# vlc-robot/robot-3dlotus

Measured on AMD Instinct MI355X. Metric: keystep-samples/sec (train fwd+bwd) 3D-LOTUS GemBench, higher is better.
Workload: dtype f32; 1 GPU; 3D-LOTUS v1 (68.18M params), 16 key-step clouds x 4096 pts per GPU, fwd+loss+bwd, train mode (dropout on), fp32 exact (MFMA f32); global_batch=16, parallelism=dp1, rccl_ranks=0

## Files before the change

### robot-3dlotus_amd/csrc/gemm.hip

```cpp
#include "gemm_common.h"
#include <stdlib.h>
#include <type_traits>

namespace LOTUS_NS {


template <int R, bool KC, int BK>
struct GTile {
  static constexpr int kLd = KC ? BK + 4 : R;
  static constexpr int kFloats = KC ? R * (BK + 4) : BK * R;
};

template <int BM, int BN, int BK, bool A_KC, bool B_KC, bool SUM_A>
__device__ __forceinline__ void gemm_slab(const float* __restrict__ As, const float* __restrict__ Bs, int wr0, int wc0,
                                          f32x16 (&acc)[BM / 64][BN / 64], float (&asum)[BM / 64]) {
  constexpr int TM = BM / 64, TN = BN / 64, KS = BK / 2;
  const int l31 = threadIdx.x & 31, h = (threadIdx.x >> 5) & 1;
  float a[TM][KS], b[TN][KS];
#pragma unroll
  for (int tm = 0; tm < TM; ++tm) {
    if (A_KC) {
      const float* row = As + (wr0 + tm * 32 + l31) * GTile<BM, true, BK>::kLd + h * KS;
#pragma unroll
      for (int q = 0; q < KS / 4; ++q) {
        const float4 v = ld4(row + 4 * q);
        a[tm][4 * q] = v.x; a[tm][4 * q + 1] = v.y; a[tm][4 * q + 2] = v.z; a[tm][4 * q + 3] = v.w;
      }
    } else {
#pragma unroll
      for (int s2 = 0; s2 < KS; ++s2) a[tm][s2] = As[(h * KS + s2) * BM + wr0 + tm * 32 + l31];
    }
  }
#pragma unroll
  for (int tn = 0; tn < TN; ++tn) {
    if (B_KC) {
      const float* row = Bs + (wc0 + tn * 32 + l31) * GTile<BN, true, BK>::kLd + h * KS;
#pragma unroll
      for (int q = 0; q < KS / 4; ++q) {
        const float4 v = ld4(row + 4 * q);
        b[tn][4 * q] = v.x; b[tn][4 * q + 1] = v.y; b[tn][4 * q + 2] = v.z; b[tn][4 * q + 3] = v.w;
      }
    } else {
#pragma unroll
      for (int s2 = 0; s2 < KS; ++s2) b[tn][s2] = Bs[(h * KS + s2) * BN + wc0 + tn * 32 + l31];
    }
  }
#pragma unroll
  for (int s2 = 0; s2 < KS; ++s2) {
#pragma unroll
    for (int tm = 0; tm < TM; ++tm) {
      if (SUM_A) asum[tm] += a[tm][s2];
#pragma unroll
      for (int tn = 0; tn < TN; ++tn) acc[tm][tn] = __builtin_amdgcn_mfma_f32_32x32x2f32(a[tm][s2], b[tn][s2], acc[tm][tn], 0, 0, 0);
    }
  }
}


__device__ __forceinline__ float4 zsel(bool ok, float4 v) {
  return make_float4(ok ? v.x : 0.f, ok ? v.y : 0.f, ok ? v.z : 0.f, ok ? v.w : 0.f);
}

template <int BM, int BN, int BK, bool A_KC, bool B_KC, bool SUM_A, bool FAST, int PREC = 0, typename EA = float, typename EB = float,
          typename EC = float, int RD = 1, bool TAP = false>
__global__ __launch_bounds__(256) void gemm_kernel(GemmP p) {
  const EA* __restrict__ pA = static_cast<const EA*>(p.A);
  const EB* __restrict__ pB = static_cast<const EB*>(p.B);
  const int* __restrict__ a_rows = TAP ? p.a_rows : nullptr;
  constexpr int TM = BM / 64, TN = BN / 64;
  constexpr int A4 = BM * BK / 4 / 256, B4 = BN * BK / 4 / 256;
  static_assert(A4 >= 1 && B4 >= 1, "tile too small");
  static_assert(PREC == 0 || ((!SUM_A || !A_KC) && BK % 16 == 0 && (A_KC || A4 % 2 == 0) && (B_KC || B4 % 2 == 0)),
                "bf16 path: operands contiguous along their non-reduction index are staged as k pairs; the bias-gradient "
                "sums are taken from the fp32 staging registers of such an A operand");
  constexpr int AF = PREC ? BTile<BM, BK, PREC>::kWords : GTile<BM, A_KC, BK>::kFloats;
  constexpr int BF = PREC ? BTile<BN, BK, PREC>::kWords : GTile<BN, B_KC, BK>::kFloats;
  constexpr int WN = BN / 2, SLD = WN + 4;
  constexpr int LDSF = (2 * AF + 2 * BF) > (4 * 32 * SLD) ? (2 * AF + 2 * BF) : (4 * 32 * SLD);
  __shared__ __attribute__((aligned(16))) float smem[LDSF];
  float* As = smem;
  float* Bs = smem + 2 * AF;

  const int tid = threadIdx.x, wave = tid >> 6;
  int bx = blockIdx.x, by = blockIdx.y, bz = blockIdx.z;
  if (gridDim.z > 1 && (gridDim.z & 7) == 0) {
    const int tiles = gridDim.x * gridDim.y;
    const int id = (blockIdx.z * gridDim.y + blockIdx.y) * gridDim.x + blockIdx.x;
    const int xcd = id & 7, slot = id >> 3;
    bz = xcd + 8 * (slot / tiles);
    const int t = slot - (slot / tiles) * tiles;
    by = t / (int)gridDim.x;
    bx = t - by * (int)gridDim.x;
  } else {
    const int nbx = gridDim.x, total = nbx * gridDim.y;
    const int lin = by * nbx + bx, xcd = lin & 7, slot = lin >> 3;
    const int q = total >> 3, r = total & 7;
    const int t = xcd * q + min(xcd, r) + slot;
    by = t / nbx;
    bx = t - by * nbx;
  }
  const int m0 = by * BM, n0 = bx * BN;
  if constexpr (TAP) {
    const int tap = m0 / p.tap_rows;
    if (m0 - tap * p.tap_rows >= p.tap_cnt[tap]) return;
    pB += (long)(p.b_tap_mirror ? 26 - tap : tap) * p.b_tap_stride;
  }
  auto arow = [&](int r) { r = min(r, p.M - 1); return TAP ? a_rows[r] : r; };
  const int kbeg = bz * p.klen;
  const int kend = min(p.K, kbeg + p.klen);
  const int wr0 = (wave >> 1) * (BM / 2), wc0 = (wave & 1) * (BN / 2);

  f32x16 acc[TM][TN];
#pragma unroll
  for (int i = 0; i < TM; ++i)
#pragma unroll
    for (int j = 0; j < TN; ++j)
#pragma unroll
      for (int r = 0; r < 16; ++r) acc[i][j][r] = 0.f;
  float asum[TM];
#pragma unroll
  for (int i = 0; i < TM; ++i) asum[i] = 0.f;

  float bsum[4] = {0.f, 0.f, 0.f, 0.f};
  Raw4<EA> rring_a[RD][A4];
  Raw4<EB> rring_b[RD][B4];
  auto gload = [&](Raw4<EA> (&rra)[A4], Raw4<EB> (&rrb)[B4], int k0) {
#pragma unroll
    for (int t = 0; t < A4; ++t) {
      const int f = tid + t * 256;
      if (A_KC) {
        const int row = f / (BK / 4), kq = f % (BK / 4);
        if (FAST) {
          const int k = k0 + kq * 4;
          rra[t] = rsel(k < kend, ldraw(pA + (long)arow(m0 + row) * p.lda + min(k, p.K - 4)));
        } else {
          rra[t] = toraw(load4_guard(pA, p.lda, m0 + row, k0 + kq * 4, p.M, kend, p.a_vec), pA);
        }
      } else {
        const int f2 = PREC ? tid + (t >> 1) * 256 : f;
        const int kr = PREC ? (f2 / (BM / 4)) * 2 + (t & 1) : f / (BM / 4), iq = f2 % (BM / 4);
        if (FAST) {
          const int k = k0 + kr;
          rra[t] = rsel(k < kend, ldraw(pA + (long)min(k, p.K - 1) * p.lda + min(m0 + iq * 4, p.M - 4)));
        } else {
          rra[t] = toraw(load4_guard(pA, p.lda, k0 + kr, m0 + iq * 4, kend, p.M, p.a_vec), pA);
        }
      }
    }
#pragma unroll
    for (int t = 0; t < B4; ++t) {
      const int f = tid + t * 256;
      if (B_KC) {
        const int row = f / (BK / 4), kq = f % (BK / 4);
        if (FAST) {
          const int k = k0 + kq * 4;
          rrb[t] = rsel(k < kend, ldraw(pB + (long)min(n0 + row, p.N - 1) * p.ldb + min(k, p.K - 4)));
        } else {
          rrb[t] = toraw(load4_guard(pB, p.ldb, n0 + row, k0 + kq * 4, p.N, kend, p.b_vec), pB);
        }
      } else {
        const int f2 = PREC ? tid + (t >> 1) * 256 : f;
        const int kr = PREC ? (f2 / (BN / 4)) * 2 + (t & 1) : f / (BN / 4), jq = f2 % (BN / 4);
        if (FAST) {
          const int k = k0 + kr;
          rrb[t] = rsel(k < kend, ldraw(pB + (long)min(k, p.K - 1) * p.ldb + min(n0 + jq * 4, p.N - 4)));
        } else {
          rrb[t] = toraw(load4_guard(pB, p.ldb, k0 + kr, n0 + jq * 4, kend, p.N, p.b_vec), pB);
        }
      }
    }
  };
  auto lstore = [&](const Raw4<EA> (&rra)[A4], const Raw4<EB> (&rrb)[B4], float* Ad, float* Bd) {
    float4 ra[A4], rb[B4];
#pragma unroll
    for (int t = 0; t < A4; ++t) ra[t] = unraw(rra[t]);
#pragma unroll
    for (int t = 0; t < B4; ++t) rb[t] = unraw(rrb[t]);
    if (PREC) {
      unsigned* Aw = reinterpret_cast<unsigned*>(Ad);
      unsigned* Bw = reinterpret_cast<unsigned*>(Bd);
      using TA = BTile<BM, BK, PREC ? PREC : 1>;
      using TB = BTile<BN, BK, PREC ? PREC : 1>;
      if (A_KC) {
#pragma unroll
        for (int t = 0; t < A4; ++t) {
          const int f = tid + t * 256, row = f / (BK / 4), kq = f % (BK / 4);
          unsigned h0, l0, h1, l1;
          split_bf16(ra[t].x, ra[t].y, h0, l0);
          split_bf16(ra[t].z, ra[t].w, h1, l1);
          *reinterpret_cast<uint2*>(&Aw[row * TA::kLdW + kq * 2]) = make_uint2(h0, h1);
          if (PREC == 3) *reinterpret_cast<uint2*>(&Aw[TA::kPlaneW + row * TA::kLdW + kq * 2]) = make_uint2(l0, l1);
        }
      } else {
#pragma unroll
        for (int t = 0; t + 1 < A4; t += 2) {
          const int f2 = tid + (t >> 1) * 256, kr2 = f2 / (BM / 4), iq = f2 % (BM / 4);
          const float va[4] = {ra[t].x, ra[t].y, ra[t].z, ra[t].w}, vb[4] = {ra[t + 1].x, ra[t + 1].y, ra[t + 1].z, ra[t + 1].w};
          unsigned hw[4], lw[4];
#pragma unroll
          for (int e = 0; e < 4; ++e) split_bf16(va[e], vb[e], hw[e], lw[e]);
          if (SUM_A && bx == 0) {
#pragma unroll
            for (int e = 0; e < 4; ++e) bsum[e] += va[e] + vb[e];
          }
          const int rot = (iq >> 2) & 3;
          rot4(hw, rot);
          if (PREC == 3) rot4(lw, rot);
#pragma unroll
          for (int e = 0; e < 4; ++e) {
            const int row = iq * 4 + ((e + rot) & 3);
            Aw[row * TA::kLdW + kr2] = hw[e];
            if (PREC == 3) Aw[TA::kPlaneW + row * TA::kLdW + kr2] = lw[e];
          }
        }
      }
      if (B_KC) {
#pragma unroll
        for (int t = 0; t < B4; ++t) {
          const int f = tid + t * 256, row = f / (BK / 4), kq = f % (BK / 4);
          unsigned h0, l0, h1, l1;
          split_bf16(rb[t].x, rb[t].y, h0, l0);
          split_bf16(rb[t].z, rb[t].w, h1, l1);
          *reinterpret_cast<uint2*>(&Bw[row * TB::kLdW + kq * 2]) = make_uint2(h0, h1);
          if (PREC == 3) *reinterpret_cast<uint2*>(&Bw[TB::kPlaneW + row * TB::kLdW + kq * 2]) = make_uint2(l0, l1);
        }
      } else {
#pragma unroll
        for (int t = 0; t + 1 < B4; t += 2) {
          const int f2 = tid + (t >> 1) * 256, kr2 = f2 / (BN / 4), jq = f2 % (BN / 4);
          const float va[4] = {rb[t].x, rb[t].y, rb[t].z, rb[t].w}, vb[4] = {rb[t + 1].x, rb[t + 1].y, rb[t + 1].z, rb[t + 1].w};
          unsigned hw[4], lw[4];
#pragma unroll
          for (int e = 0; e < 4; ++e) split_bf16(va[e], vb[e], hw[e], lw[e]);
          const int rot = (jq >> 2) & 3;
          rot4(hw, rot);
          if (PREC == 3) rot4(lw, rot);
#pragma unroll
          for (int e = 0; e < 4; ++e) {
            const int row = jq * 4 + ((e + rot) & 3);
            Bw[row * TB::kLdW + kr2] = hw[e];
            if (PREC == 3) Bw[TB::kPlaneW + row * TB::kLdW + kr2] = lw[e];
          }
        }
      }
      return;
    }
#pragma unroll
    for (int t = 0; t < A4; ++t) {
      const int f = tid + t * 256;
      const float v[4] = {ra[t].x, ra[t].y, ra[t].z, ra[t].w};
      if (A_KC) {
        const int row = f / (BK / 4), kq = f % (BK / 4);
        st4(&Ad[row * GTile<BM, true, BK>::kLd + kq * 4], ra[t]);
      } else {
        const int kr = f / (BM / 4), iq = f % (BM / 4);
        st4(&Ad[kr * BM + iq * 4], ra[t]);
      }
    }
#pragma unroll
    for (int t = 0; t < B4; ++t) {
      const int f = tid + t * 256;
      const float v[4] = {rb[t].x, rb[t].y, rb[t].z, rb[t].w};
      if (B_KC) {
        const int row = f / (BK / 4), kq = f % (BK / 4);
        st4(&Bd[row * GTile<BN, true, BK>::kLd + kq * 4], rb[t]);
      } else {
        const int kr = f / (BN / 4), jq = f % (BN / 4);
        st4(&Bd[kr * BN + jq * 4], rb[t]);
      }
    }
  };

  const EA* pa[A4];
  const EB* pb[B4];
  if (FAST) {
#pragma unroll
    for (int t = 0; t < A4; ++t) {
      const int f = tid + t * 256;
      if (A_KC) pa[t] = pA + (long)arow(m0 + f / (BK / 4)) * p.lda + (f % (BK / 4)) * 4;
      else if (PREC) pa[t] = pA + (long)(((tid + (t >> 1) * 256) / (BM / 4)) * 2 + (t & 1)) * p.lda + min(m0 + ((tid + (t >> 1) * 256) % (BM / 4)) * 4, p.M - 4);
      else pa[t] = pA + (long)(f / (BM / 4)) * p.lda + min(m0 + (f % (BM / 4)) * 4, p.M - 4);
    }
#pragma unroll
    for (int t = 0; t < B4; ++t) {
      const int f = tid + t * 256;
      if (B_KC) pb[t] = pB + (long)min(n0 + f / (BK / 4), p.N - 1) * p.ldb + (f % (BK / 4)) * 4;
      else if (PREC) pb[t] = pB + (long)(((tid + (t >> 1) * 256) / (BN / 4)) * 2 + (t & 1)) * p.ldb + min(n0 + ((tid + (t >> 1) * 256) % (BN / 4)) * 4, p.N - 4);
      else pb[t] = pB + (long)(f / (BN / 4)) * p.ldb + min(n0 + (f % (BN / 4)) * 4, p.N - 4);
    }
  }
  auto gload_full = [&](Raw4<EA> (&rra)[A4], Raw4<EB> (&rrb)[B4], int k0) {
#pragma unroll
    for (int t = 0; t < A4; ++t) rra[t] = ldraw(pa[t] + (A_KC ? (long)k0 : (long)k0 * p.lda));
#pragma unroll
    for (int t = 0; t < B4; ++t) rrb[t] = ldraw(pb[t] + (B_KC ? (long)k0 : (long)k0 * p.ldb));
  };

  auto slab = [&](int cur) {
    if (PREC) gemm_slab_bf16<BM, BN, BK, PREC ? PREC : 1>(reinterpret_cast<const unsigned*>(As + cur * AF), reinterpret_cast<const unsigned*>(Bs + cur * BF), wr0, wc0, acc);
    else if (SUM_A && bx == 0) gemm_slab<BM, BN, BK, A_KC, B_KC, true>(As + cur * AF, Bs + cur * BF, wr0, wc0, acc, asum);
    else gemm_slab<BM, BN, BK, A_KC, B_KC, false>(As + cur * AF, Bs + cur * BF, wr0, wc0, acc, asum);
  };
  auto simple_loop = [&]() {
    gload(rring_a[0], rring_b[0], kbeg);
    lstore(rring_a[0], rring_b[0], As, Bs);
    __syncthreads();
    int cur = 0;
    for (int k0 = kbeg; k0 < kend; k0 += BK) {
      if (FAST && k0 + 2 * BK <= kend) gload_full(rring_a[0], rring_b[0], k0 + BK);
      else gload(rring_a[0], rring_b[0], k0 + BK);
      __builtin_amdgcn_sched_barrier(0);
      slab(cur);
      __builtin_amdgcn_sched_barrier(0);
      cur ^= 1;
      lstore(rring_a[0], rring_b[0], As + cur * AF, Bs + cur * BF);
      __syncthreads();
    }
  };
  if constexpr (RD == 1 || !FAST) {
    if (kbeg < kend) simple_loop();
  } else if (kend - kbeg < RD * BK) {
    if (kbeg < kend) simple_loop();
  } else {
#pragma unroll
    for (int d = 0; d < RD; ++d) gload_full(rring_a[d], rring_b[d], kbeg + d * BK);
    lstore(rring_a[0], rring_b[0], As, Bs);
    __syncthreads();
    int cur = 0, k0 = kbeg;
    for (; k0 + 2 * RD * BK <= kend; k0 += RD * BK) {
#pragma unroll
      for (int d = 0; d < RD; ++d) {
        gload_full(rring_a[d], rring_b[d], k0 + (d + RD) * BK);
        __builtin_amdgcn_sched_barrier(0);
        slab(cur);
        __builtin_amdgcn_sched_barrier(0);
        cur ^= 1;
        lstore(rring_a[(d + 1) % RD], rring_b[(d + 1) % RD], As + cur * AF, Bs + cur * BF);
        __syncthreads();
      }
    }
#pragma unroll
    for (int d = 0; d < 2 * RD; ++d) {
      const int kk = k0 + d * BK;
      if (kk < kend) {
        if (d < RD && kk + RD * BK < kend) {
          if (kk + (RD + 1) * BK <= kend) gload_full(rring_a[d], rring_b[d], kk + RD * BK);
          else gload(rring_a[d], rring_b[d], kk + RD * BK);
        }
        __builtin_amdgcn_sched_barrier(0);
        slab(cur);
        __builtin_amdgcn_sched_barrier(0);
        cur ^= 1;
        if (kk + BK < kend) lstore(rring_a[(d + 1) % RD], rring_b[(d + 1) % RD], As + cur * AF, Bs + cur * BF);
        __syncthreads();
      }
    }
  }

  const bool fused = FAST && p.cnt != nullptr && gridDim.z > 1;
  EC* __restrict__ C = static_cast<EC*>(p.C) + (long)bz * p.part_stride;
  float* __restrict__ Cp = fused ? p.part + (long)bz * p.part_stride : nullptr;
  if (FAST) {
    float* st = smem + wave * (32 * SLD);
    const int l31 = tid & 31, hh = (tid >> 5) & 1, lane = tid & 63;
    constexpr int LPR = WN / 4;
    constexpr int RPI = 64 / LPR;
    __syncthreads();
#pragma unroll
    for (int tm = 0; tm < TM; ++tm) {
#pragma unroll
      for (int tn = 0; tn < TN; ++tn)
#pragma unroll
        for (int r = 0; r < 16; ++r) st[((r & 3) + 8 * (r >> 2) + 4 * hh) * SLD + tn * 32 + l31] = acc[tm][tn][r];
      __syncthreads();
      const int c4 = lane % LPR;
      const int col = n0 + wc0 + c4 * 4;
      if (col < p.N) {
#pragma unroll
        for (int it = 0; it < 32 / RPI; ++it) {
          const int rl = it * RPI + lane / LPR;
          const int row = m0 + wr0 + tm * 32 + rl;
          if (row < p.M) {
            const long o = (long)row * p.ldc + col;
            const float4 a4 = ld4(st + rl * SLD + c4 * 4);
            if (fused) {
              st_agent4(Cp + o, a4);
            } else {
              float v[4] = {a4.x, a4.y, a4.z, a4.w};
              gemm_epilogue4(p, C, o, col, v);
            }
          }
        }
      }
      __syncthreads();
    }
  } else {
#pragma unroll
    for (int tm = 0; tm < TM; ++tm)
#pragma unroll
      for (int tn = 0; tn < TN; ++tn) {
        const int col = n0 + acc_col(wc0, tn);
        if (col >= p.N) continue;
        const float bv = p.bias ? p.bias[col] : 0.f;
#pragma unroll
        for (int r = 0; r < 16; ++r) {
          const int row = m0 + acc_row(wr0, tm, r);
          if (row >= p.M) continue;
          const long o = (long)row * p.ldc + col;
          float v = acc[tm][tn][r] + bv;
          if (p.pre) st1(p.pre + o, v);
          v = act_f(v, p.act);
          if (p.mulpre) v *= act_grad_f(ld1(p.mulpre + o), p.dact);
          if (p.drop_thresh) v *= dropout_scale(p.drop_seed, (unsigned long long)o, p.drop_thresh, p.drop_inv_keep);
          if (p.residual) v += ld1(p.residual + o);
          st1(C + o, v);
        }
      }
  }
  if (SUM_A && PREC) {
    __syncthreads();
    if (p.bias_part && bx == 0) {
      float4* red = reinterpret_cast<float4*>(smem);
      red[tid] = make_float4(bsum[0], bsum[1], bsum[2], bsum[3]);
      __syncthreads();
      if (tid < BM) {
        constexpr int G = 256 / (BM / 4);
        float sacc = 0.f;
#pragma unroll
        for (int g = 0; g < G; ++g) {
          const float4 v = red[g * (BM / 4) + (tid >> 2)];
          sacc += (tid & 3) == 0 ? v.x : (tid & 3) == 1 ? v.y : (tid & 3) == 2 ? v.z : v.w;
        }
        if (m0 + tid < p.M) __hip_atomic_store(p.bias_part + (long)bz * p.bias_stride + m0 + tid, sacc, __ATOMIC_RELAXED, __HIP_MEMORY_SCOPE_AGENT);
      }
    }
  } else if (SUM_A) {
    if (p.bias_part && bx == 0 && (wave & 1) == 0) {
#pragma unroll
      for (int tm = 0; tm < TM; ++tm) {
        float s = asum[tm] + __shfl_xor(asum[tm], 32, 64);
        const int i = m0 + wr0 + tm * 32 + (tid & 31);
        if ((tid & 32) == 0 && i < p.M) __hip_atomic_store(p.bias_part + (long)bz * p.bias_stride + i, s, __ATOMIC_RELAXED, __HIP_MEMORY_SCOPE_AGENT);
      }
    }
  }
  if (FAST && fused) splitk_fused_tail<SUM_A, BM, BN, EC>(p, bx, by, m0, n0, tid);
}

template <typename T>
__global__ __launch_bounds__(256) void reduce_parts_kernel(const T* __restrict__ part, T* __restrict__ out, long n,
                                                           long stride, int nz, int accumulate) {
  __shared__ float4 red[16][16];
  const int q = threadIdx.x & 15, zl = threadIdx.x >> 4;
  const long e = ((long)blockIdx.x * 16 + q) * 4;
  float4 s = make_float4(0.f, 0.f, 0.f, 0.f);
  if (e + 3 < n) {
    for (int z = zl; z < nz; z += 16) {
      const float4 v = ld4(part + (long)z * stride + e);
      s.x += v.x; s.y += v.y; s.z += v.z; s.w += v.w;
    }
  } else if (e < n) {
    float t[4] = {0.f, 0.f, 0.f, 0.f};
    for (int z = zl; z < nz; z += 16)
      for (int k = 0; k < 4 && e + k < n; ++k) t[k] += ld1(part + (long)z * stride + e + k);
    s = make_float4(t[0], t[1], t[2], t[3]);
  }
  red[zl][q] = s;
  __syncthreads();
  if (zl == 0 && e < n) {
    float4 t = red[0][q];
    for (int k = 1; k < 16; ++k) {
      t.x += red[k][q].x; t.y += red[k][q].y; t.z += red[k][q].z; t.w += red[k][q].w;
    }
    const float tv[4] = {t.x, t.y, t.z, t.w};
    for (int k = 0; k < 4 && e + k < n; ++k) st1(out + e + k, accumulate ? ld1(out + e + k) + tv[k] : tv[k]);
  }
}

int lotus_reduce_parts(const float* part, float* out, long n, long stride, int nz, int accumulate, hipStream_t st) {
  if (n <= 0) return LOTUS_OK;
  LOTUS_LAUNCH(reduce_parts_kernel<float>, dim3(cdiv(n, 64)), dim3(256), 0, st, part, out, n, stride, nz, accumulate);
  LOTUS_LAUNCH_CHECK("lotus_reduce_parts");
  return LOTUS_OK;
}

extern "C" int lotus_sum_slabs(const act_t* part, act_t* out, long n, long stride, int nz, void* stream) {
  LOTUS_CHECK_ARG(part && out && n >= 0 && nz >= 1, "lotus_sum_slabs: bad arguments");
  if (n <= 0) return LOTUS_OK;
  LOTUS_LAUNCH(reduce_parts_kernel<act_t>, dim3(cdiv(n, 64)), dim3(256), 0, (hipStream_t)stream, part, out, n, stride, nz, 0);
  LOTUS_LAUNCH_CHECK("lotus_sum_slabs");
  return LOTUS_OK;
}

__global__ __launch_bounds__(256) void sum_slabs_ld_kernel(const act_t* __restrict__ part, act_t* __restrict__ out, int rows, int cols,
                                                           long out_ld, long stride, int nz) {
  const int c4 = cols / 4;
  const long i = (long)blockIdx.x * 256 + threadIdx.x;
  if (i >= (long)rows * c4) return;
  const int r = (int)(i / c4), q = (int)(i % c4);
  const act_t* src = part + (long)r * cols + 4 * q;
  float4 s = ld4(src);
  int z = 1;
  for (; z + 3 < nz; z += 4) {
    const float4 v0 = ld4(src + (long)z * stride), v1 = ld4(src + (long)(z + 1) * stride);
    const float4 v2 = ld4(src + (long)(z + 2) * stride), v3 = ld4(src + (long)(z + 3) * stride);
    s.x = (((s.x + v0.x) + v1.x) + v2.x) + v3.x; s.y = (((s.y + v0.y) + v1.y) + v2.y) + v3.y;
    s.z = (((s.z + v0.z) + v1.z) + v2.z) + v3.z; s.w = (((s.w + v0.w) + v1.w) + v2.w) + v3.w;
  }
  for (; z < nz; ++z) {
    const float4 v = ld4(src + (long)z * stride);
    s.x += v.x; s.y += v.y; s.z += v.z; s.w += v.w;
  }
  st4(out + (long)r * out_ld + 4 * q, s);
}

extern "C" int lotus_sum_slabs_ld(const act_t* part, act_t* out, int rows, int cols, long out_ld, long stride, int nz, void* stream) {
  LOTUS_CHECK_ARG(part && out && rows >= 0 && cols > 0 && cols % 4 == 0 && out_ld % 4 == 0 && stride % 4 == 0 && nz >= 1,
                  "lotus_sum_slabs_ld: bad arguments (cols, out_ld and stride must be multiples of 4)");
  if (rows == 0) return LOTUS_OK;
  LOTUS_LAUNCH(sum_slabs_ld_kernel, dim3(cdiv((long)rows * (cols / 4), 256)), dim3(256), 0, (hipStream_t)stream, part, out, rows, cols,
               out_ld, stride, nz);
  LOTUS_LAUNCH_CHECK("lotus_sum_slabs_ld");
  return LOTUS_OK;
}

static inline int vec_ok(const void* p, long ld) { return (((uintptr_t)p) % 16 == 0) && (ld % 4 == 0); }

#define GEMM_KALIGN 64

#define GEMM_GO_RD(BM_, BN_, BK_, PREC_, grid_, RD_)                                                                             \
  do {                                                                                                                           \
    using TB_ = std::conditional_t<SUM_A, act_t, float>;                                                                         \
                            \
    auto note_ = [&] { lotus_note_dense_route(1, BM_, BN_, BK_, nz, FAST, FAST && p.cnt && nz > 1, RD_); };                      \
    if constexpr (LOTUS_ACT_IS_BF16 && !SUM_A) {                                                                                 \
      if (p.b_act) {                       \
        if constexpr (PREC_ == 1 && FAST) {                                                                                      \
          note_();                                                                                                               \
          if (p.c_float) LOTUS_LAUNCH((gemm_kernel<BM_, BN_, BK_, A_KC, B_KC, SUM_A, FAST, PREC_, act_t, act_t, float, RD_>), grid_, block, 0, st, p); \
          else LOTUS_LAUNCH((gemm_kernel<BM_, BN_, BK_, A_KC, B_KC, SUM_A, FAST, PREC_, act_t, act_t, act_t, RD_>), grid_, block, 0, st, p); \
        }                                                                                                                        \
      } else if (p.c_float) {                                                                                                    \
        note_();                                                                                                                 \
        LOTUS_LAUNCH((gemm_kernel<BM_, BN_, BK_, A_KC, B_KC, SUM_A, FAST, PREC_, act_t, TB_, float, RD_>), grid_, block, 0, st, p); \
      } else {                                                                                                                   \
        note_();                                                                                                                 \
        LOTUS_LAUNCH((gemm_kernel<BM_, BN_, BK_, A_KC, B_KC, SUM_A, FAST, PREC_, act_t, TB_, act_t, RD_>), grid_, block, 0, st, p); \
      }                                                                                                                          \
    } else {                                                                                                                     \
      note_();                                                                                                                   \
      LOTUS_LAUNCH((gemm_kernel<BM_, BN_, BK_, A_KC, B_KC, SUM_A, FAST, PREC_, act_t, TB_, float, RD_>), grid_, block, 0, st, p);      \
    }                                                                                                                            \
  } while (0)
#define GEMM_GO(BM_, BN_, BK_, PREC_, grid_) GEMM_GO_RD(BM_, BN_, BK_, PREC_, grid_, 1)

constexpr long kF32RingMaxBlocks = 8192;
constexpr int kBf16RingMaxRows = 8192;

template <bool A_KC, bool B_KC, bool SUM_A, bool FAST>
static int launch_gemm_t(GemmP& p, int nz, hipStream_t st) {
  const long blocks64 = (long)cdiv(p.M, 64) * cdiv(p.N, 64);
  dim3 block(256);
  dim3 g64(cdiv(p.N, 64), cdiv(p.M, 64), nz);
  const int g_prec = p.prec;
  if (g_prec && SUM_A && FAST && !A_KC && !B_KC) {
    if constexpr (SUM_A && !A_KC && !B_KC && FAST) {
      if (g_prec == 1) {
        if constexpr (LOTUS_ACT_IS_BF16) {
          if (p.K <= kBf16RingMaxRows) GEMM_GO_RD(64, 64, 32, 1, g64, 4);
          else GEMM_GO(64, 64, 32, 1, g64);
        } else {
          GEMM_GO(64, 64, 32, 1, g64);
        }
      } else if constexpr (!LOTUS_ACT_IS_BF16) GEMM_GO(64, 64, 32, 3, g64);
    }
    LOTUS_LAUNCH_CHECK("lotus_gemm(bf16 wgrad)");
    return LOTUS_OK;
  }
  if (p.b_act && !(LOTUS_ACT_IS_BF16 && g_prec == 1 && !SUM_A && FAST && (A_KC || p.M % 4 == 0))) {
    lotus_set_error("lotus_linear: bf16 weight shadows (precision 5) need the bf16-storage build and 16-byte aligned operands whose "
                    "widths are multiples of 4");
    return LOTUS_E_UNSUPPORTED;
  }
  if (g_prec && !SUM_A && FAST && (A_KC || p.M % 4 == 0)) {
    if constexpr (!SUM_A && FAST) {
      if (g_prec == 1) {
        if constexpr (LOTUS_ACT_IS_BF16) {
          if (p.M <= kBf16RingMaxRows) GEMM_GO_RD(64, 64, 32, 1, g64, 4);
          else GEMM_GO(64, 64, 32, 1, g64);
        } else GEMM_GO(64, 64, 32, 1, g64);
      } else if constexpr (!LOTUS_ACT_IS_BF16) {
        GEMM_GO(64, 64, 32, 3, g64);
      }
    }
    LOTUS_LAUNCH_CHECK("lotus_gemm(bf16)");
    return LOTUS_OK;
  }
  if constexpr (LOTUS_ACT_IS_BF16) {
    GEMM_GO(64, 64, 32, 0, g64);
  } else {
    const long blocks_eff = p.tap_rows ? blocks64 / 2 : blocks64;
    const int bk = SUM_A ? 32 : (blocks_eff * nz <= 512 ? 64 : (blocks_eff * nz <= 2048 ? 32 : 16));
    const int rd = SUM_A ? 1 : (blocks_eff * nz <= kF32RingMaxBlocks ? 2 : 1);
    if (p.tap_rows) {
      if constexpr (A_KC && !SUM_A && FAST && !LOTUS_ACT_IS_BF16) {
        lotus_note_dense_route(1, 64, 64, bk, nz, FAST, 0, 2);
        if (bk == 64) LOTUS_LAUNCH((gemm_kernel<64, 64, 64, A_KC, B_KC, SUM_A, FAST, 0, act_t, float, float, 2, true>), g64, block, 0, st, p);
        else if (bk == 32) LOTUS_LAUNCH((gemm_kernel<64, 64, 32, A_KC, B_KC, SUM_A, FAST, 0, act_t, float, float, 2, true>), g64, block, 0, st, p);
        else LOTUS_LAUNCH((gemm_kernel<64, 64, 16, A_KC, B_KC, SUM_A, FAST, 0, act_t, float, float, 2, true>), g64, block, 0, st, p);
        LOTUS_LAUNCH_CHECK("lotus_gemm(tap-grouped)");
        return LOTUS_OK;
      } else {
        lotus_set_error("lotus_gemm: tap-grouped products need k-contiguous, 16-byte aligned fp32 rows");
        return LOTUS_E_UNSUPPORTED;
      }
    }
    if (rd == 2 && bk == 64) GEMM_GO_RD(64, 64, 64, 0, g64, 2);
    else if (rd == 2 && bk == 16) GEMM_GO_RD(64, 64, 16, 0, g64, 2);
    else if (rd == 2) GEMM_GO_RD(64, 64, 32, 0, g64, 2);
    else if (bk == 64) GEMM_GO(64, 64, 64, 0, g64);
    else if (bk == 32) GEMM_GO(64, 64, 32, 0, g64);
    else GEMM_GO(64, 64, 16, 0, g64);
  }
  LOTUS_LAUNCH_CHECK("lotus_gemm");
  return LOTUS_OK;
}

template <bool A_KC, bool B_KC>
static bool fast_ok(const GemmP& p) {
  const bool a_ok = p.a_vec && (A_KC ? (p.K % 4 == 0 && p.K >= 4) : (p.M % 4 == 0 && p.M >= 4));
  const bool b_ok = p.b_vec && (B_KC ? (p.K % 4 == 0 && p.K >= 4) : (p.N % 4 == 0 && p.N >= 4));
  const bool c_ok = p.N % 4 == 0 && p.ldc % 4 == 0 && p.part_stride % 4 == 0 && vec_ok(p.C, p.ldc) &&
                    (!p.bias || ((uintptr_t)p.bias) % 16 == 0) && (!p.residual || ((uintptr_t)p.residual) % 16 == 0) &&
                    (!p.pre || ((uintptr_t)p.pre) % 16 == 0) && (!p.mulpre || ((uintptr_t)p.mulpre) % 16 == 0) &&
                    (!p.part || ((uintptr_t)p.part) % 16 == 0);
  return a_ok && b_ok && c_ok;
}

template <bool A_KC, bool B_KC, bool SUM_A>
static int launch_gemm(GemmP& p, int nz, hipStream_t st) {
  const bool a_ok = p.a_vec && (A_KC ? (p.K % 4 == 0 && p.K >= 4) : (p.M % 4 == 0 && p.M >= 4));
  const bool b_ok = p.b_vec && (B_KC ? (p.K % 4 == 0 && p.K >= 4) : (p.N % 4 == 0 && p.N >= 4));
  const bool c_ok = p.N % 4 == 0 && p.ldc % 4 == 0 && p.part_stride % 4 == 0 && vec_ok(p.C, p.ldc) &&
                    (!p.bias || ((uintptr_t)p.bias) % 16 == 0) && (!p.residual || ((uintptr_t)p.residual) % 16 == 0) &&
                    (!p.pre || ((uintptr_t)p.pre) % 16 == 0) && (!p.mulpre || ((uintptr_t)p.mulpre) % 16 == 0);
  if (a_ok && b_ok && c_ok) {
    if constexpr (A_KC || SUM_A) {
      const int rc = launch_gemm_dma(p, A_KC ? (B_KC ? 0 : 1) : 2, nz, st);
      if (rc != LOTUS_GEMM_DMA_NA) return rc;
    }
    return launch_gemm_t<A_KC, B_KC, SUM_A, true>(p, nz, st);
  }
  return launch_gemm_t<A_KC, B_KC, SUM_A, false>(p, nz, st);
}

static void set_drop(GemmP& p, float drop_p, unsigned long long seed) {
  p.drop_seed = seed;
  lotus_drop_setup(drop_p, &p.drop_thresh, &p.drop_inv_keep);
}

__global__ void splitk_epilogue_kernel(GemmP p, const float* __restrict__ part, long stride, int nz) {
  const int n4 = p.N / 4;
  const long total4 = (long)p.M * n4;
  for (long i = (long)blockIdx.x * blockDim.x + threadIdx.x; i < total4; i += (long)gridDim.x * blockDim.x) {
    const int row = (int)(i / n4), col = (int)(i % n4) * 4;
    const long o = (long)row * p.ldc + col;
    float4 s4 = ld4(part + o);
    for (int z = 1; z < nz; ++z) {
      const float4 v = ld4(part + (long)z * stride + o);
      s4.x += v.x; s4.y += v.y; s4.z += v.z; s4.w += v.w;
    }
    float v[4] = {s4.x, s4.y, s4.z, s4.w};
    if (p.bias) {
      const float4 b = ld4(p.bias + col);
      v[0] += b.x; v[1] += b.y; v[2] += b.z; v[3] += b.w;
    }
    if (p.pre) st4(p.pre + o, make_float4(v[0], v[1], v[2], v[3]));
#pragma unroll
    for (int e = 0; e < 4; ++e) v[e] = act_f(v[e], p.act);
    if (p.mulpre) {
      const float4 m4 = ld4(p.mulpre + o);
      const float mv[4] = {m4.x, m4.y, m4.z, m4.w};
#pragma unroll
      for (int e = 0; e < 4; ++e) v[e] *= act_grad_f(mv[e], p.dact);
    }
    if (p.drop_thresh) {
      float dm[4];
      dropout_scale4(p.drop_seed, (unsigned long long)o, p.drop_thresh, p.drop_inv_keep, dm);
#pragma unroll
      for (int e = 0; e < 4; ++e) v[e] *= dm[e];
    }
    if (p.residual) {
      const float4 r4 = ld4(p.residual + o);
      v[0] += r4.x; v[1] += r4.y; v[2] += r4.z; v[3] += r4.w;
    }
    st4(static_cast<act_t*>(p.C) + o, make_float4(v[0], v[1], v[2], v[3]));
  }
}

static int fwd_splits(int M, int N, int K) {
  const long blocks = (long)cdiv(M, 64) * cdiv(N, 64);
  int nz = 1;
  while (nz < 16 && blocks * nz < 512 && K / (nz * 2) >= 384) nz *= 2;
  return nz;
}

#define LOTUS_SPLITK_MAX_TILES 4096

static bool splitk_fused_enabled() {
  static int on = -1;
  if (on < 0) { const char* e = getenv("LOTUS_SPLITK_FUSED"); on = (e && e[0] == '0') ? 0 : 1; }
  return on != 0;
}

template <bool A_KC, bool B_KC>
static int run_gemm_splitk(GemmP& p, void* workspace, size_t workspace_bytes, unsigned* counters, hipStream_t st) {
  if (!splitk_fused_enabled()) counters = nullptr;
  const int nz = (p.N % 4 == 0 && p.ldc == p.N) ? fwd_splits(p.M, p.N, p.K) : 1;
  const size_t need = (size_t)nz * p.M * p.N * sizeof(float);
  if (nz == 1 || !workspace || workspace_bytes < need || ((uintptr_t)workspace) % 16) return launch_gemm<A_KC, B_KC, false>(p, 1, st);
  const int klen = cdiv(cdiv(p.K, nz), GEMM_KALIGN) * GEMM_KALIGN;
  const long tiles = (long)cdiv(p.M, 64) * cdiv(p.N, 64);
  if (counters && tiles <= LOTUS_SPLITK_MAX_TILES) {
    GemmP q = p;
    q.part = (float*)workspace; q.part_stride = (long)p.M * p.N; q.cnt = counters; q.klen = klen;
    if (fast_ok<A_KC, B_KC>(q)) return launch_gemm<A_KC, B_KC, false>(q, nz, st);
  }
  GemmP q = p;
  q.C = workspace; q.c_float = 1; q.part_stride = (long)p.M * p.N;
  q.bias = nullptr; q.residual = nullptr; q.pre = nullptr; q.mulpre = nullptr; q.act = LOTUS_ACT_NONE; q.drop_thresh = 0;
  q.klen = klen;
  StopEventOnLast stop_ev;
  int rc = launch_gemm<A_KC, B_KC, false>(q, nz, st);
  if (rc) return rc;
  const long total4 = (long)p.M * p.N / 4;
  int g = cdiv(total4, 256);
  stop_ev.last();
  LOTUS_LAUNCH(splitk_epilogue_kernel, dim3(g > 2048 ? 2048 : g), dim3(256), 0, st, p, (const float*)workspace,
                     (long)p.M * p.N, nz);
  LOTUS_LAUNCH_CHECK("lotus_gemm(split-K epilogue)");
  return LOTUS_OK;
}

int lotus_conv_tap_gemm(int mode, const act_t* x, const float* w, float* part, const int* tg_in, const int* tg_cnt, int n64,
                        int src_rows, int cin, int cout, hipStream_t st) {
  if constexpr (LOTUS_ACT_IS_BF16) {
    return LOTUS_E_UNSUPPORTED;
  } else {
    GemmP p;
    memset(&p, 0, sizeof(p));
    p.A = x; p.B = w; p.C = part;
    p.M = 27 * n64;
    p.N = mode == 0 ? cout : cin;
    p.K = mode == 0 ? cin : cout;
    p.lda = p.K; p.ldb = 27L * cin; p.ldc = p.N;
    p.act = LOTUS_ACT_NONE;
    p.klen = cdiv(p.K, GEMM_KALIGN) * GEMM_KALIGN;
    p.a_vec = vec_ok(x, p.K); p.b_vec = vec_ok(w, cin) && cin % 4 == 0; p.prec = 0;
    p.drop_inv_keep = 1.f;
    p.a_rows = tg_in; p.tap_cnt = tg_cnt; p.tap_rows = n64; p.b_tap_mirror = mode == 1; p.b_tap_stride = cin;
    p.a_src_rows = src_rows;
    {
      GemmP q = p;
      const int rc = launch_gemm_dma_tap(q, mode, st);
      if (rc != LOTUS_GEMM_DMA_NA) return rc;
    }
    if (!(fast_ok<true, true>(p))) {
      lotus_set_error("lotus_subm_conv(tap-grouped): rows, weights and the partial slab must be 16-byte aligned with widths that are multiples of 4");
      return LOTUS_E_UNSUPPORTED;
    }
    return mode == 0 ? launch_gemm<true, true, false>(p, 1, st) : launch_gemm<true, false, false>(p, 1, st);
  }
}

extern "C" {

size_t lotus_splitk_counters_bytes(void) { return (size_t)(LOTUS_SPLITK_MAX_TILES + 64) * sizeof(unsigned); }
size_t lotus_bn_counters_offset(void) { return (size_t)LOTUS_SPLITK_MAX_TILES * sizeof(unsigned); }

size_t lotus_linear_workspace(int M, int N, int K) {
  const int a = fwd_splits(M, N, K), b = fwd_splits(M, K, N);
  const size_t wa = a > 1 ? (size_t)a * M * N * sizeof(float) : 0, wb = b > 1 ? (size_t)b * M * K * sizeof(float) : 0;
  return wa > wb ? wa : wb;
}

int lotus_linear_fwd(const act_t* x, const float* w, const float* bias, const act_t* residual, act_t* y,
                     act_t* pre, int M, int N, int K, int act, float drop_p, unsigned long long drop_seed,
                     int precision, void* workspace, size_t workspace_bytes, void* counters, void* stream) {
  LOTUS_CHECK_ARG(x && w && y && M >= 0 && N > 0 && K > 0, "lotus_linear_fwd: bad arguments");
  const int w_shadow = precision == 5;
  LOTUS_CHECK_ARG(!w_shadow || LOTUS_ACT_IS_BF16, "lotus_linear_fwd: precision 5 (bf16 weight shadow) exists in the bf16-storage build only");
  if (w_shadow) precision = 1;
  LOTUS_CHECK_ARG(precision == 0 || precision == 1 || precision == 3, "lotus_linear_fwd: precision must be 0, 1 or 3 (5 with bf16 weights)");
  LOTUS_CHECK_ARG(!(LOTUS_ACT_IS_BF16 && precision == 3), "lotus_linear_fwd: bf16x3 operands (precision 3) are not built for bf16 activation storage; use 1 (bf16) or 0");
  if (M == 0) return LOTUS_OK;
  GemmP p;
  memset(&p, 0, sizeof(p));
  p.A = x; p.B = w; p.C = y; p.M = M; p.N = N; p.K = K;
  p.lda = K; p.ldb = K; p.ldc = N;
  p.bias = bias; p.residual = residual; p.pre = pre; p.act = act;
  p.klen = cdiv(K, GEMM_KALIGN) * GEMM_KALIGN;
  p.a_vec = vec_ok(x, K); p.b_vec = vec_ok(w, K); p.prec = precision; p.b_act = w_shadow;
  set_drop(p, drop_p, drop_seed);
  return run_gemm_splitk<true, true>(p, workspace, workspace_bytes, (unsigned*)counters, (hipStream_t)stream);
}

int lotus_linear_dgrad(const act_t* dy, const float* w, act_t* dx, const act_t* pre, const act_t* add, int M,
                       int N, int K, int act, float drop_p, unsigned long long drop_seed, int precision, void* workspace,
                       size_t workspace_bytes, void* counters, void* stream) {
  LOTUS_CHECK_ARG(dy && w && dx && M >= 0 && N > 0 && K > 0, "lotus_linear_dgrad: bad arguments");
  const int w_shadow = precision == 5;
  LOTUS_CHECK_ARG(!w_shadow || LOTUS_ACT_IS_BF16, "lotus_linear_dgrad: precision 5 (bf16 weight shadow) exists in the bf16-storage build only");
  if (w_shadow) precision = 1;
  LOTUS_CHECK_ARG(precision == 0 || precision == 1 || precision == 3, "lotus_linear_dgrad: precision must be 0, 1 or 3 (5 with bf16 weights)");
  LOTUS_CHECK_ARG(!(LOTUS_ACT_IS_BF16 && precision == 3), "lotus_linear_dgrad: bf16x3 operands (precision 3) are not built for bf16 activation storage; use 1 (bf16) or 0");
  if (M == 0) return LOTUS_OK;
  GemmP p;
  memset(&p, 0, sizeof(p));
  p.A = dy; p.B = w; p.C = dx; p.M = M; p.N = K; p.K = N;
  p.lda = N; p.ldb = K; p.ldc = K;
  p.act = LOTUS_ACT_NONE;
  p.mulpre = pre; p.dact = act; p.residual = add;
  p.klen = cdiv(N, GEMM_KALIGN) * GEMM_KALIGN;
  p.a_vec = vec_ok(dy, N); p.b_vec = vec_ok(w, K); p.prec = precision; p.b_act = w_shadow;
  set_drop(p, drop_p, drop_seed);
  return run_gemm_splitk<true, false>(p, workspace, workspace_bytes, (unsigned*)counters, (hipStream_t)stream);
}

int lotus_layernorm_bwd(const act_t* dy, const act_t* x, const float* mean, const float* rstd, const float* gamma, const act_t* add,
                        act_t* dx, float* dgamma, float* dbeta, int M, int C, int accumulate, act_t* dz, float drop_p,
                        unsigned long long drop_seed, void* workspace, size_t workspace_bytes, void* stream);
int lotus_layernorm_bwd_parts(int M, int C);
int lotus_linear_dgrad_ln(const act_t* dy, const float* w, const act_t* x, const float* mean, const float* rstd, const float* gamma,
                          const act_t* add, act_t* dx, act_t* dn, act_t* dz, float dz_p, unsigned long long dz_seed, int M, int N,
                          int K, int precision, void* workspace, size_t workspace_bytes, void* counters, void* ln_workspace,
                          size_t ln_workspace_bytes, int* nparts, void* stream) {
  LOTUS_CHECK_ARG(dy && w && x && mean && rstd && gamma && dx && dn && nparts && ln_workspace && M >= 0 && N > 0 && K > 0,
                  "lotus_linear_dgrad_ln: bad arguments");
  LOTUS_CHECK_ARG(!dz || dz_p > 0.f, "lotus_linear_dgrad_ln: dz needs dz_p > 0");
  if (M == 0) { *nparts = 0; return LOTUS_OK; }
  if (precision == 0 && !LOTUS_ACT_IS_BF16 && (size_t)cdiv(M, 128) * 2 * K * sizeof(float) <= ln_workspace_bytes) {
    GemmP p;
    memset(&p, 0, sizeof(p));
    p.A = dy; p.B = w; p.C = dx; p.M = M; p.N = K; p.K = N;
    p.lda = N; p.ldb = K; p.ldc = K;
    p.act = LOTUS_ACT_NONE; p.residual = add;
    p.klen = cdiv(N, GEMM_KALIGN) * GEMM_KALIGN;
    p.a_vec = vec_ok(dy, N); p.b_vec = vec_ok(w, K); p.prec = 0;
    set_drop(p, dz ? dz_p : 0.f, dz_seed);
    p.ln_x = x; p.ln_mean = mean; p.ln_rstd = rstd; p.ln_gamma = gamma; p.ln_part = (float*)ln_workspace; p.ln_dz = dz;
    if (p.a_vec && p.b_vec && vec_ok(dx, K) && vec_ok(x, K) && (!add || vec_ok(add, K))) {
      const int rc = launch_gemm_dma(p, 1, 1, (hipStream_t)stream);
      if (rc != LOTUS_GEMM_DMA_NA) { *nparts = cdiv(M, 128); return rc; }
    }
  }
  StopEventOnLast stop_ev;
  int rc = lotus_linear_dgrad(dy, w, dn, nullptr, nullptr, M, N, K, LOTUS_ACT_NONE, 0.f, 0, precision, workspace, workspace_bytes, counters, stream);
  if (rc) return rc;
  stop_ev.last();
  rc = lotus_layernorm_bwd(dn, x, mean, rstd, gamma, add, dx, nullptr, nullptr, M, K, 0, dz, dz ? dz_p : 0.f, dz_seed, ln_workspace,
                           ln_workspace_bytes, stream);
  *nparts = lotus_layernorm_bwd_parts(M, K);
  return rc;
}

int lotus_dense_last_route(int* out) {
  LOTUS_CHECK_ARG(out, "lotus_dense_last_route: out is null");
  for (int i = 0; i < 8; ++i) out[i] = lotus_tls_dense_route[i];
  return LOTUS_OK;
}

static int wgrad_splits(int M, int N, int K) {
  if (const int dz = gemm_dma_wgrad_splits(M, N, K)) return dz;
  int nz = 1;
  const long tiles = (long)cdiv(N, 64) * cdiv(K, 64);
  if (tiles >= 128 && M < 1024) return 1;
  while (nz < 256 && tiles * nz < 1024 && M / (nz * 2) >= 128) nz *= 2;
  return nz;
}

size_t lotus_linear_wgrad_workspace(int M, int N, int K) {
  return (size_t)wgrad_splits(M, N, K) * ((size_t)N * K + N) * sizeof(float);
}

int lotus_linear_wgrad(const act_t* dy, const act_t* x, float* dw, float* db, int M, int N, int K,
                       int accumulate, int precision, void* workspace, size_t workspace_bytes, void* counters,
                       void* stream) {
  LOTUS_CHECK_ARG(dy && x && dw && M >= 0 && N > 0 && K > 0, "lotus_linear_wgrad: bad arguments");
  if (precision == 5) precision = 1;
  LOTUS_CHECK_ARG(precision == 0 || precision == 1 || precision == 3, "lotus_linear_wgrad: precision must be 0, 1 or 3");
  LOTUS_CHECK_ARG(!(LOTUS_ACT_IS_BF16 && precision == 3), "lotus_linear_wgrad: bf16x3 operands (precision 3) are not built for bf16 activation storage; use 1 (bf16) or 0");
  hipStream_t st = (hipStream_t)stream;
  const int nz = wgrad_splits(M, N, K);
  const size_t slab = (size_t)N * K + N;
  LOTUS_CHECK_ARG(workspace && workspace_bytes >= (size_t)nz * slab * sizeof(float),
                  "lotus_linear_wgrad: workspace too small (%zu < %zu)", workspace_bytes, (size_t)nz * slab * sizeof(float));
  const bool direct = nz == 1 && !accumulate;
  float* part = (float*)workspace;
  GemmP p;
  memset(&p, 0, sizeof(p));
  p.A = dy; p.B = x; p.M = N; p.N = K; p.K = M;
  p.lda = N; p.ldb = K; p.ldc = K;
  p.klen = cdiv(cdiv(M > 0 ? M : 1, nz), GEMM_KALIGN) * GEMM_KALIGN;
  p.a_vec = vec_ok(dy, N); p.b_vec = vec_ok(x, K); p.prec = precision;
  set_drop(p, 0.f, 0);
  constexpr int fuse_max = 4;
  const long wtiles = (long)cdiv(N, 64) * cdiv(K, 64);
  if (!direct && counters && splitk_fused_enabled() && nz > 1 && nz <= fuse_max && wtiles <= LOTUS_SPLITK_MAX_TILES) {
    GemmP q = p;
    q.C = dw; q.part = part; q.part_stride = (long)slab; q.cnt = (unsigned*)counters;
    q.bias_part = db ? part + (size_t)N * K : nullptr; q.bias_stride = (long)slab; q.bias_out = db; q.accumulate = accumulate;
    if (fast_ok<false, false>(q)) return launch_gemm<false, false, true>(q, nz, st);
  }
  if (direct) {
    p.C = dw; p.bias_part = db;
  } else {
    p.C = part; p.part_stride = (long)slab;
    p.bias_part = db ? part + (size_t)N * K : nullptr; p.bias_stride = (long)slab;
  }
  int rc = launch_gemm<false, false, true>(p, nz, st);
  if (rc || direct) return rc;
  const long n = (long)N * K;
  if (db && db == dw + n) return lotus_reduce_parts(part, dw, (long)slab, (long)slab, nz, accumulate, st);
  rc = lotus_reduce_parts(part, dw, n, (long)slab, nz, accumulate, st);
  if (!rc && db) rc = lotus_reduce_parts(part + n, db, (long)N, (long)slab, nz, accumulate, st);
  return rc;
}

}

}
```

Baseline: 1094 keystep-samples/s.

## Adapt split-K partial reduction layout to slab count with batched loads

The split-K partial-sum reduction kernel is templated on how many threads split the slab dimension (2/4/8/16) and how many column groups each thread handles. A host dispatcher picks the variant from nz and n. Loads are issued in unrolled batches of up to 8 independent float4 reads before accumulating. This targets the old fixed 16x16 layout, which idled most threads when nz was small and serialised its loads. The cost is more template instantiations and code size, and a different summation order that may perturb fp32 results slightly.

```diff
diff --git a/robot-3dlotus_amd/csrc/gemm.hip b/robot-3dlotus_amd/csrc/gemm.hip
--- a/robot-3dlotus_amd/csrc/gemm.hip
+++ b/robot-3dlotus_amd/csrc/gemm.hip
@@ -447,39 +447,127 @@
   if (FAST && fused) splitk_fused_tail<SUM_A, BM, BN, EC>(p, bx, by, m0, n0, tid);
 }
 
-template <typename T>
+template <typename T, bool TAIL>
+__device__ __forceinline__ float4 rp_load(const T* p, int rem) {
+  if (!TAIL) return ld4(p);
+  return make_float4(ld1(p), rem > 1 ? ld1(p + 1) : 0.f, rem > 2 ? ld1(p + 2) : 0.f, 0.f);
+}
+
+template <typename T, int R, bool TAIL>
+__device__ __forceinline__ void rp_batch(float4& s, const T* col, long stride, int z0, int zsafe, int nz, int rem) {
+  float4 v[R];
+#pragma unroll
+  for (int k = 0; k < R; ++k) {
+    const int z = z0 + 16 * k;
+    v[k] = rp_load<T, TAIL>(col + (long)(z < nz ? z : zsafe) * stride, rem);
+  }
+#pragma unroll
+  for (int k = 0; k < R; ++k) {
+    if (z0 + 16 * k < nz) { s.x += v[k].x; s.y += v[k].y; s.z += v[k].z; s.w += v[k].w; }
+  }
+}
+
+template <typename T, bool TAIL>
+__device__ __forceinline__ float4 rp_lane_sum(const T* col, long stride, int zl, int nz, int rem) {
+  float4 s = make_float4(0.f, 0.f, 0.f, 0.f);
+  if (zl >= nz) return s;
+  int steps = (nz + 15) / 16;
+  int z = zl;
+  for (; steps >= 8; steps -= 8, z += 128) rp_batch<T, 8, TAIL>(s, col, stride, z, zl, nz, rem);
+  switch (steps) {
+    case 7: rp_batch<T, 7, TAIL>(s, col, stride, z, zl, nz, rem); break;
+    case 6: rp_batch<T, 6, TAIL>(s, col, stride, z, zl, nz, rem); break;
+    case 5: rp_batch<T, 5, TAIL>(s, col, stride, z, zl, nz, rem); break;
+    case 4: rp_batch<T, 4, TAIL>(s, col, stride, z, zl, nz, rem); break;
+    case 3: rp_batch<T, 3, TAIL>(s, col, stride, z, zl, nz, rem); break;
+    case 2: rp_batch<T, 2, TAIL>(s, col, stride, z, zl, nz, rem); break;
+    case 1: rp_batch<T, 1, TAIL>(s, col, stride, z, zl, nz, rem); break;
+    default: break;
+  }
+  return s;
+}
+
+template <typename T, int R, int CPT>
+__device__ __forceinline__ void rp_batch_cols(float4 (&s)[CPT], const T* col, long colstep, long stride, int z0, int zsafe, int nz) {
+  float4 v[R][CPT];
+#pragma unroll
+  for (int k = 0; k < R; ++k) {
+    const int z = z0 + 16 * k;
+    const T* p = col + (long)(z < nz ? z : zsafe) * stride;
+#pragma unroll
+    for (int j = 0; j < CPT; ++j) v[k][j] = ld4(p + j * colstep);
+  }
+#pragma unroll
+  for (int k = 0; k < R; ++k) {
+    if (z0 + 16 * k < nz) {
+#pragma unroll
+      for (int j = 0; j < CPT; ++j) { s[j].x += v[k][j].x; s[j].y += v[k][j].y; s[j].z += v[k][j].z; s[j].w += v[k][j].w; }
+    }
+  }
+}
+
+template <typename T, int ZL, int CPT>
 __global__ __launch_bounds__(256) void reduce_parts_kernel(const T* __restrict__ part, T* __restrict__ out, long n,
                                                            long stride, int nz, int accumulate) {
-  __shared__ float4 red[16][16];
-  const int q = threadIdx.x & 15, zl = threadIdx.x >> 4;
-  const long e = ((long)blockIdx.x * 16 + q) * 4;
-  float4 s = make_float4(0.f, 0.f, 0.f, 0.f);
-  if (e + 3 < n) {
-    for (int z = zl; z < nz; z += 16) {
-      const float4 v = ld4(part + (long)z * stride + e);
-      s.x += v.x; s.y += v.y; s.z += v.z; s.w += v.w;
-    }
-  } else if (e < n) {
-    float t[4] = {0.f, 0.f, 0.f, 0.f};
-    for (int z = zl; z < nz; z += 16)
-      for (int k = 0; k < 4 && e + k < n; ++k) t[k] += ld1(part + (long)z * stride + e + k);
-    s = make_float4(t[0], t[1], t[2], t[3]);
-  }
-  red[zl][q] = s;
+  constexpr int COLS = 256 / ZL, BC = COLS * CPT;
+  __shared__ float4 red[ZL][BC];
+  const int q = threadIdx.x % COLS, zl = threadIdx.x / COLS;
+  const long e0 = ((long)blockIdx.x * BC + q) * 4;
+  float4 s[CPT];
+#pragma unroll
+  for (int j = 0; j < CPT; ++j) s[j] = make_float4(0.f, 0.f, 0.f, 0.f);
+  if (CPT > 1 && e0 + (CPT - 1) * COLS * 4 + 3 < n) {
+    if (zl < nz) {
+      constexpr int RMAX = 8 / CPT;
+      int steps = (nz + 15) / 16, z = zl;
+      for (; steps >= RMAX; steps -= RMAX, z += 16 * RMAX) rp_batch_cols<T, RMAX, CPT>(s, part + e0, COLS * 4, stride, z, zl, nz);
+      if (RMAX > 2 && steps >= 2) { rp_batch_cols<T, 2, CPT>(s, part + e0, COLS * 4, stride, z, zl, nz); steps -= 2; z += 32; }
+      if (steps >= 1) rp_batch_cols<T, 1, CPT>(s, part + e0, COLS * 4, stride, z, zl, nz);
+    }
+  } else {
+#pragma unroll
+    for (int j = 0; j < CPT; ++j) {
+      const long e = e0 + (long)j * COLS * 4;
+      if (e + 3 < n) s[j] = rp_lane_sum<T, false>(part + e, stride, zl, nz, 4);
+      else if (e < n) s[j] = rp_lane_sum<T, true>(part + e, stride, zl, nz, (int)(n - e));
+    }
+  }
+#pragma unroll
+  for (int j = 0; j < CPT; ++j) red[zl][q + j * COLS] = s[j];
   __syncthreads();
-  if (zl == 0 && e < n) {
-    float4 t = red[0][q];
-    for (int k = 1; k < 16; ++k) {
-      t.x += red[k][q].x; t.y += red[k][q].y; t.z += red[k][q].z; t.w += red[k][q].w;
+  for (int c = threadIdx.x; c < BC; c += 256) {
+    const long e = ((long)blockIdx.x * BC + c) * 4;
+    if (e >= n) break;
+    float4 t = red[0][c];
+#pragma unroll
+    for (int k = 1; k < ZL; ++k) {
+      t.x += red[k][c].x; t.y += red[k][c].y; t.z += red[k][c].z; t.w += red[k][c].w;
     }
     const float tv[4] = {t.x, t.y, t.z, t.w};
     for (int k = 0; k < 4 && e + k < n; ++k) st1(out + e + k, accumulate ? ld1(out + e + k) + tv[k] : tv[k]);
   }
 }
 
+template <typename T, int ZL>
+static void launch_reduce_parts_zl(const T* part, T* out, long n, long stride, int nz, int accumulate, hipStream_t st) {
+  constexpr long BE = 4 * (256 / ZL);
+  const int steps = cdiv(nz, 16);
+  if (steps <= 2 && n >= 4 * BE * 256) LOTUS_LAUNCH((reduce_parts_kernel<T, ZL, 4>), dim3(cdiv(n, 4 * BE)), dim3(256), 0, st, part, out, n, stride, nz, accumulate);
+  else if (steps <= 4 && n >= 2 * BE * 256) LOTUS_LAUNCH((reduce_parts_kernel<T, ZL, 2>), dim3(cdiv(n, 2 * BE)), dim3(256), 0, st, part, out, n, stride, nz, accumulate);
+  else LOTUS_LAUNCH((reduce_parts_kernel<T, ZL, 1>), dim3(cdiv(n, BE)), dim3(256), 0, st, part, out, n, stride, nz, accumulate);
+}
+
+template <typename T>
+static void launch_reduce_parts(const T* part, T* out, long n, long stride, int nz, int accumulate, hipStream_t st) {
+  if (nz > 8) launch_reduce_parts_zl<T, 16>(part, out, n, stride, nz, accumulate, st);
+  else if (nz > 4) launch_reduce_parts_zl<T, 8>(part, out, n, stride, nz, accumulate, st);
+  else if (nz > 2) launch_reduce_parts_zl<T, 4>(part, out, n, stride, nz, accumulate, st);
+  else launch_reduce_parts_zl<T, 2>(part, out, n, stride, nz, accumulate, st);
+}
+
 int lotus_reduce_parts(const float* part, float* out, long n, long stride, int nz, int accumulate, hipStream_t st) {
   if (n <= 0) return LOTUS_OK;
-  LOTUS_LAUNCH(reduce_parts_kernel<float>, dim3(cdiv(n, 64)), dim3(256), 0, st, part, out, n, stride, nz, accumulate);
+  launch_reduce_parts<float>(part, out, n, stride, nz, accumulate, st);
   LOTUS_LAUNCH_CHECK("lotus_reduce_parts");
   return LOTUS_OK;
 }
@@ -487,7 +575,7 @@
 extern "C" int lotus_sum_slabs(const act_t* part, act_t* out, long n, long stride, int nz, void* stream) {
   LOTUS_CHECK_ARG(part && out && n >= 0 && nz >= 1, "lotus_sum_slabs: bad arguments");
   if (n <= 0) return LOTUS_OK;
-  LOTUS_LAUNCH(reduce_parts_kernel<act_t>, dim3(cdiv(n, 64)), dim3(256), 0, (hipStream_t)stream, part, out, n, stride, nz, 0);
+  launch_reduce_parts<act_t>(part, out, n, stride, nz, 0, (hipStream_t)stream);
   LOTUS_LAUNCH_CHECK("lotus_sum_slabs");
   return LOTUS_OK;
 }
```

After: 1098 keystep-samples/s, median of 4. Within noise of the previous version (+0.4%).
